# meyerls/FruitNeRF

Measured on AMD Instinct MI355X. Metric: train rays/sec, fruit_nerf on synthetic apple 800x800, higher is better.
Workload: dtype f32 fwd (MLP GEMMs: 3-piece bf16 split, 6 products, ~2^-24) / 2-piece bwd (dX, dW: 3 products, ~2^-17; its forward recompute 3-piece); everything else f32

## Files before the change

fruitnerf_amd/csrc/hash_scatter.hip:

```cpp
#include <stdlib.h>
#include <string.h>

#include "hash_sources.hpp"
#include "sequencer.hpp"

namespace fnr {

constexpr int SC_MAX_ROWS = 8192;
constexpr int SC_MAX_BINS = 256;
constexpr int SC_CHUNK = 512;
constexpr int SC_EMIT_THREADS = 512;
constexpr int SC_PER_THREAD = SC_CHUNK / SC_EMIT_THREADS;
constexpr int SC_BINS_PER_THREAD = 1;
static_assert(SC_MAX_BINS <= SC_EMIT_THREADS, "one bin per thread");
constexpr int SC_CNT_STRIDE = 32;

__device__ unsigned long long g_scatter_overflow_records;
__device__ unsigned long long g_scatter_records[2][64][16];



struct ScatterPlan {
  int log2_rows;
  int bins_per_level;
// ... 62 lines not shown
  const unsigned long long heads = __ballot(head);
  const uint32_t row = (uint32_t)(heads >> (lane & 48)) & 0xffffu;
  const uint32_t below = row & ((2u << j) - 1u);
  const int dist = j - (31 - __clz((int)below));
  RunMasks m;
  m.g1 = dist >= 1 ? 1.0f : 0.0f;
  m.g2 = dist >= 2 ? 1.0f : 0.0f;
  m.g4 = dist >= 4 ? 1.0f : 0.0f;
  m.g8 = dist >= 8 ? 1.0f : 0.0f;
  m.tail = (j == 15) || ((row >> (j + 1)) & 1u);
  m.any_run = ~heads != 0ull;
  return m;
}
__device__ __forceinline__ float run_sum(float v, const RunMasks& m) {
  v = fmaf(m.g1, dpp_shr0_f32<0x111>(v), v);
  v = fmaf(m.g2, dpp_shr0_f32<0x112>(v), v);
  v = fmaf(m.g4, dpp_shr0_f32<0x114>(v), v);
  v = fmaf(m.g8, dpp_shr0_f32<0x118>(v), v);
  return v;
}



template <class Source, bool PAIRS>
__global__ __launch_bounds__(SC_EMIT_THREADS) void k_scatter_emit(GridDev grid, Warp warp, Source src, long long N,
                                                      const float2* __restrict__ d_feats, float2* __restrict__ queue_v,
                                                      unsigned short* __restrict__ queue_r, unsigned* __restrict__ qcount, unsigned* __restrict__ qmax,
                                                      long long cap, int log2_rows, int level0, int level_count, int lpb
                                                      ) {
  __shared__ float2 s_val[SC_CHUNK * 8];
  __shared__ unsigned s_key[SC_CHUNK * 8];
  __shared__ unsigned s_cnt[SC_MAX_BINS];
  __shared__ unsigned s_off[SC_MAX_BINS];
  __shared__ unsigned s_base[SC_MAX_BINS];
  __shared__ unsigned s_max;
  __shared__ unsigned s_wsum[SC_EMIT_THREADS / 64];
  const int bins = 1 << (grid.log2_T - log2_rows);
  const int lane = threadIdx.x & 63, wave = threadIdx.x >> 6;
  const uint32_t mask = (1u << grid.log2_T) - 1u;
  const uint32_t row_mask = (1u << log2_rows) - 1u;
  const long long n0 = (long long)blockIdx.x * SC_CHUNK;
  static_assert(SC_PER_THREAD == 1, "one sample per thread");
  const long long n = n0 + threadIdx.x;
  const bool valid = n < N;
  float x[3] = {0.f, 0.f, 0.f};
  float2 gf_next = make_float2(0.f, 0.f);
  const int lrel0 = blockIdx.y * lpb;
  if (valid) {
    gf_next = ntc_load<NT_DFEATS_LD>(&d_feats[(size_t)(level0 + lrel0) * N + n]);
    float px, py, pz;
    src.position(n, px, py, pz);
    warp_position(warp, px, py, pz, x);
  }
  for (int li = 0; li < lpb && lrel0 + li < level_count; ++li) {
  const int lrel = lrel0 + li;
  const int level = level0 + lrel;
  for (int i = threadIdx.x; i < bins; i += SC_EMIT_THREADS) {
    s_cnt[i] = 0;
  }
  if (threadIdx.x == 0) s_max = 0;
  __syncthreads();
  const int scaling = grid.scalings[level];
  const float2 gf = gf_next;
  if (valid && li + 1 < lpb && lrel + 1 < level_count) gf_next = ntc_load<NT_DFEATS_LD>(&d_feats[(size_t)(level + 1) * N + n]);

  uint32_t hk[SC_PER_THREAD][8];
  float vxk[SC_PER_THREAD][8], vyk[SC_PER_THREAD][8];
  float tmax = 0.0f;
  unsigned emit_mask[SC_PER_THREAD];
#pragma unroll
// ... 110 lines not shown
  __syncthreads();
  float* table = reinterpret_cast<float*>(grid.table + ((size_t)level << grid.log2_T));
  unsigned overflowed_here = 0;
  for (unsigned i = threadIdx.x; i < total; i += SC_EMIT_THREADS) {
    const float2 v = s_val[i];
    const unsigned key = s_key[i];
    const unsigned bin = key >> 16, row_in_bin = key & 0xffffu;
    const unsigned slot = s_base[bin] + (i - s_off[bin]);
    if ((long long)slot < cap) {
      const size_t q = ((size_t)lrel * bins + bin) * cap + slot;
      queue_v[q] = v;
      queue_r[q] = (unsigned short)row_in_bin;
    } else {
      qmax[(size_t)lrel * SC_CNT_STRIDE + 1] = 1u;
      ++overflowed_here;
      const size_t row = ((size_t)bin << log2_rows) + row_in_bin;
      atomicAdd(table + 2 * row, v.x);
      atomicAdd(table + 2 * row + 1, v.y);
    }
  }
  if (overflowed_here) atomicAdd(&g_scatter_overflow_records, (unsigned long long)overflowed_here);
  __syncthreads();
  }
}

__device__ __forceinline__ void acc_record(unsigned long long* __restrict__ s_acc, unsigned row, const float2& v,
                                           double scale) {
  const long long ix = __double2ll_rn((double)v.x * scale), iy = __double2ll_rn((double)v.y * scale);
  atomicAdd(&s_acc[2 * row], (unsigned long long)ix);
  atomicAdd(&s_acc[2 * row + 1], (unsigned long long)iy);
}

struct AccArgs {
  GridDev grid;
  const float2* queue_v;
  const unsigned short* queue_r;
  unsigned *qcount, *qmax, *qdone;
  long long cap;
  int log2_rows, level0, nbins;
  int kind;
  TableAdam adam;
};

template <bool ADAM>
__device__ __forceinline__ void accumulate_bin(const AccArgs& A, int vblock, unsigned long long* __restrict__ s_acc) {
  const GridDev& grid = A.grid;
// ... 121 lines not shown
        const int pair = e2 >> 1;
        if (!((tw1[pair >> 5] >> (pair & 31)) & 1u)) atomicOr(&tw1[pair >> 5], 1u << (pair & 31));
      }
      float2 P = adam.p[row0 + e2], M = adam.m[row0 + e2], V = adam.v[row0 + e2];
      table_adam_update(adam, g.x, P.x, M.x, V.x);
      table_adam_update(adam, g.y, P.y, M.y, V.y);
      adam.p[row0 + e2] = P;
      adam.m[row0 + e2] = M;
      adam.v[row0 + e2] = V;
    }
  } else {
    for (int e2 = threadIdx.x; e2 < rows; e2 += blockDim.x) {
      const long long ax = (long long)s_acc[2 * e2], ay = (long long)s_acc[2 * e2 + 1];
      if (ax != 0 || ay != 0) {
        float2 t = dst[e2];
        t.x += (float)((double)ax * inv);
        t.y += (float)((double)ay * inv);
        dst[e2] = t;
      }
    }
  }
}

extern __shared__ __attribute__((aligned(16))) unsigned char acc_smem[];
template <bool ADAM>
__global__ __launch_bounds__(1024) void k_scatter_accumulate(AccArgs a) {
  accumulate_bin<ADAM>(a, (int)blockIdx.x, reinterpret_cast<unsigned long long*>(acc_smem));
}
template <bool ADAM>
__global__ __launch_bounds__(1024) void k_scatter_accumulate2(AccArgs a, AccArgs b) {
  unsigned long long* s_acc = reinterpret_cast<unsigned long long*>(acc_smem);
  if ((int)blockIdx.x < a.nbins) accumulate_bin<ADAM>(a, (int)blockIdx.x, s_acc);
  else accumulate_bin<ADAM>(b, (int)blockIdx.x - a.nbins, s_acc);
}


template <class Source>
static int scatter_emit(const fnr_grid* grid_grad, const Warp& warp, const Source& src, long long N,
                        const float2* d_feats, int level0, int level_count, void* workspace, size_t workspace_bytes,
                        int workspace_clean, hipStream_t st, const TableAdam* adam, AccArgs& acc) {
  FNR_CHECK_ARG(level0 >= 0 && level_count >= 1 && level0 + level_count <= grid_grad->n_levels,
                "hash scatter: level range [%d,+%d) outside the %d levels", level0, level_count, grid_grad->n_levels);
  const ScatterPlan p = scatter_plan(N, level_count, grid_grad->log2_hashmap_size);
  FNR_CHECK_ARG(p.bins_per_level <= SC_MAX_BINS, "hash scatter: log2_hashmap_size %d too large for the bin histogram",
                grid_grad->log2_hashmap_size);
  FNR_CHECK_ARG(workspace && workspace_bytes >= p.count_bytes + p.queue_bytes, "hash scatter: workspace too small");
  unsigned* qcount = reinterpret_cast<unsigned*>(workspace);
  float2* queue_v = reinterpret_cast<float2*>(reinterpret_cast<char*>(workspace) + p.count_bytes);
  unsigned short* queue_r = reinterpret_cast<unsigned short*>(reinterpret_cast<char*>(workspace) + p.count_bytes + p.value_bytes);
  if (!workspace_clean) FNR_HIP(hipMemsetAsync(qcount, 0, p.count_bytes, st));
  const size_t nbins_all = (size_t)level_count * p.bins_per_level;
  const long long chunks = (N + SC_CHUNK - 1) / SC_CHUNK;
  FNR_CHECK_ARG(chunks < (1ll << 31), "hash scatter: too many samples");
  const GridDev gd = make_grid(grid_grad);
  for (int l = 0; l < grid_grad->n_levels; ++l)
    FNR_CHECK_ARG(gd.scalings[l] > 0 && gd.scalings[l] < 65535, "hash scatter: level resolution %d out of range", gd.scalings[l]);
  bool pairs = true;
  for (int l = level0; l < level0 + level_count; ++l) pairs = pairs && gd.scalings[l] < (1 << p.log2_rows);
  int lpb = 1;
  {
    const char* e = getenv("FNR_EMIT_LPB");
    const int forced = e ? atoi(e) : 0;
    const long long slots = 3ll * device_cu_count();
    while (lpb < level_count && lpb < 8 && chunks * ((level_count + 2 * lpb - 1) / (2 * lpb)) >= 2 * slots) lpb *= 2;
    if (forced > 0) lpb = forced;
    if (lpb > level_count) lpb = level_count;
  }
  const unsigned gy = (unsigned)((level_count + lpb - 1) / lpb);
  if (chunks == 0) {
  } else if (pairs)
    hipLaunchKernelGGL((k_scatter_emit<Source, true>), dim3((unsigned)chunks, gy), dim3(SC_EMIT_THREADS),
                       0, st, gd, warp, src, N, d_feats, queue_v, queue_r, qcount, qcount + nbins_all * SC_CNT_STRIDE, p.cap,
                       p.log2_rows, level0, level_count, lpb);
  else
    hipLaunchKernelGGL((k_scatter_emit<Source, false>), dim3((unsigned)chunks, gy), dim3(SC_EMIT_THREADS),
                       0, st, gd, warp, src, N, d_feats, queue_v, queue_r, qcount, qcount + nbins_all * SC_CNT_STRIDE, p.cap,
                       p.log2_rows, level0, level_count, lpb);
  FNR_LAUNCH_CHECK();
  acc.grid = gd;
  acc.queue_v = queue_v, acc.queue_r = queue_r, acc.qcount = qcount;
  acc.qmax = qcount + nbins_all * SC_CNT_STRIDE;
  acc.qdone = qcount + (nbins_all + level_count) * SC_CNT_STRIDE;
  acc.cap = p.cap, acc.log2_rows = p.log2_rows, acc.level0 = level0;
  acc.nbins = level_count * p.bins_per_level;
  acc.kind = 0;
  acc.adam = adam ? *adam : TableAdam{};
  return FNR_OK;
}

static int acc_lds_bytes(const AccArgs& a) { return (2 << a.log2_rows) * (int)sizeof(unsigned long long); }

static int scatter_accumulate(const AccArgs& a, bool adam, hipStream_t st) {
  const int bytes = acc_lds_bytes(a);
  if (adam) {
    const int rc = ensure_dyn_lds<k_scatter_accumulate<true>>(2 * SC_MAX_ROWS * (int)sizeof(unsigned long long));
    if (rc) return rc;
    hipLaunchKernelGGL(k_scatter_accumulate<true>, dim3((unsigned)a.nbins), dim3(1024), bytes, st, a);
  } else {
    const int rc = ensure_dyn_lds<k_scatter_accumulate<false>>(2 * SC_MAX_ROWS * (int)sizeof(unsigned long long));
    if (rc) return rc;
    hipLaunchKernelGGL(k_scatter_accumulate<false>, dim3((unsigned)a.nbins), dim3(1024), bytes, st, a);
  }
  FNR_LAUNCH_CHECK();
  return FNR_OK;
}

static int scatter_accumulate2(const AccArgs& a, const AccArgs& b, bool adam, hipStream_t st) {
  const int bytes = acc_lds_bytes(a) > acc_lds_bytes(b) ? acc_lds_bytes(a) : acc_lds_bytes(b);
  if (adam) {
    const int rc = ensure_dyn_lds<k_scatter_accumulate2<true>>(2 * SC_MAX_ROWS * (int)sizeof(unsigned long long));
    if (rc) return rc;
    hipLaunchKernelGGL(k_scatter_accumulate2<true>, dim3((unsigned)(a.nbins + b.nbins)), dim3(1024), bytes, st, a, b);
  } else {
    const int rc = ensure_dyn_lds<k_scatter_accumulate2<false>>(2 * SC_MAX_ROWS * (int)sizeof(unsigned long long));
    if (rc) return rc;
    hipLaunchKernelGGL(k_scatter_accumulate2<false>, dim3((unsigned)(a.nbins + b.nbins)), dim3(1024), bytes, st, a, b);
  }
  FNR_LAUNCH_CHECK();
  return FNR_OK;
}

template <class Source>
static int binned_scatter(const fnr_grid* grid_grad, const Warp& warp, const Source& src, long long N,
                          const float2* d_feats, int level0, int level_count, void* workspace, size_t workspace_bytes,
                          int workspace_clean, hipStream_t st, const TableAdam* adam = nullptr) {
  AccArgs acc;
  const int rc = scatter_emit(grid_grad, warp, src, N, d_feats, level0, level_count, workspace, workspace_bytes,
                              workspace_clean, st, adam, acc);
  if (rc) return rc;
  return scatter_accumulate(acc, adam != nullptr, st);
}

constexpr int PROP_PART = 320;

template <int L, int H, bool POSGRAD>
__global__ __launch_bounds__(256) void k_prop_bwd(GridDev grid, float4* __restrict__ d_xw, Warp warp, RaySource src,
                                                  long long N, const float* __restrict__ w0,
                                                  const float* __restrict__ b0, const float* __restrict__ w1,
                                                  const float* __restrict__ b1, const float2* __restrict__ feat_save,
                                                  const float* __restrict__ d_density, float2* __restrict__ d_feats,
                                                  float* __restrict__ partials) {
  constexpr int K = 2 * L;
  __shared__ float s_dh[256][H + 1];
  __shared__ float s_ha[256][H + 1];
  __shared__ float s_f[256][K + 1];
  __shared__ float s_do[256];
  static_assert(H == 16 && K <= 16, "phase 2 is a single 16x16 MFMA tile");
  using f32x4 = __attribute__((ext_vector_type(4))) float;
  const int tid = threadIdx.x;
  const int lane = tid & 63, wave = tid >> 6;
  const int j = lane & 15, g = lane >> 4;
  f32x4 d1 = {0.f, 0.f, 0.f, 0.f}, d2 = {0.f, 0.f, 0.f, 0.f}, d3 = {0.f, 0.f, 0.f, 0.f};
  float db1 = 0.0f;
  const float ones_col0 = (j == 0) ? 1.0f : 0.0f;
  const long long n_iter = (N + 255) / 256;
  for (long long it = blockIdx.x; it < n_iter; it += gridDim.x) {
    const long long n = it * 256 + tid;
    float f[K], dout = 0.0f;
#pragma unroll
    for (int k = 0; k < K; ++k) f[k] = 0.0f;
    bool sel = false;
    float x[3] = {0.f, 0.f, 0.f};
    if (n < N) {
      float px, py, pz;
      src.position(n, px, py, pz);
      sel = warp_position(warp, px, py, pz, x);
#pragma unroll
      for (int l = 0; l < L; ++l) {
        const float2 v = ntc_load<NT_PROP_FEATS>(&feat_save[(size_t)l * N + n]);
        f[2 * l] = v.x;
        f[2 * l + 1] = v.y;
      }
    }
    float a[H];
    float out = b1[0];
#pragma unroll
    for (int o = 0; o < H; ++o) {
      float t = b0[o];
#pragma unroll
// ... 56 lines not shown
      const float bf = (j < K) ? s_f[row][j < K ? j : 0] : 0.0f;
      d1 = __builtin_amdgcn_mfma_f32_16x16x4f32(a1, bf, d1, 0, 0, 0);
      d2 = __builtin_amdgcn_mfma_f32_16x16x4f32(a2, ones_col0, d2, 0, 0, 0);
      d3 = __builtin_amdgcn_mfma_f32_16x16x4f32(a1, ones_col0, d3, 0, 0, 0);
    }
    __syncthreads();
  }
  float* red = &s_dh[0][0];
#pragma unroll
  for (int r = 0; r < 4; ++r) {
    red[((wave * 3 + 0) * 16 + 4 * g + r) * 16 + j] = d1[r];
    red[((wave * 3 + 1) * 16 + 4 * g + r) * 16 + j] = d2[r];
    red[((wave * 3 + 2) * 16 + 4 * g + r) * 16 + j] = d3[r];
  }
  db1 = wave_sum(db1);
  if (lane == 0) s_do[wave] = db1;
  __syncthreads();
  {
    const int o = tid >> 4, k = tid & 15;
    auto total = [&](int which) {
      return (red[((0 * 3 + which) * 16 + o) * 16 + k] + red[((1 * 3 + which) * 16 + o) * 16 + k]) +
             (red[((2 * 3 + which) * 16 + o) * 16 + k] + red[((3 * 3 + which) * 16 + o) * 16 + k]);
    };
    float* part = partials + (size_t)blockIdx.x * PROP_PART;
    part[tid] = total(0);
    if (k == 0) {
      part[256 + o] = total(1);
      part[272 + o] = total(2);
    }
    if (tid == 0) part[288] = (s_do[0] + s_do[1]) + (s_do[2] + s_do[3]);
  }
}

constexpr int PRD_E = 16, PRD_Y = 64;
struct PropReduceArgs {
  const float* partials;
  int nblocks, K;
  float *g_w0, *g_b0, *g_w1, *g_b1;
  WeightAdam wa;
};
template <bool ADAM>
__device__ __forceinline__ void prop_reduce_block(int block, const PropReduceArgs& a) {
  __shared__ float s_part[PRD_Y][PRD_E];
  const float* __restrict__ partials = a.partials;
  const int nblocks = a.nblocks, K = a.K;
  const int t = threadIdx.x % PRD_E, y = threadIdx.x / PRD_E;
  const int e = block * PRD_E + t;
  float s = 0.0f;
  if (e <= 288) {
    int b = y;
    for (; b + 7 * PRD_Y < nblocks; b += 8 * PRD_Y) {
      float v[8];
#pragma unroll
      for (int u = 0; u < 8; ++u) v[u] = partials[(size_t)(b + u * PRD_Y) * PROP_PART + e];
#pragma unroll
      for (int u = 0; u < 8; ++u) s += v[u];
    }
    for (; b < nblocks; b += PRD_Y) s += partials[(size_t)b * PROP_PART + e];
  }
  s_part[y][t] = s;
  __syncthreads();
  if (y != 0 || e > 288) return;
#pragma unroll 8
  for (int q = 1; q < PRD_Y; ++q) s += s_part[q][t];
  if (!ADAM && s == 0.0f) return;
  float* dst = nullptr;
  if (e < 256) {
    const int o = e >> 4, k = e & 15;
    if (k < K) dst = &a.g_w0[o * K + k];
  } else if (e < 272) {
    dst = &a.g_w1[e - 256];
  } else if (e < 288) {
    dst = &a.g_b0[e - 272];
  } else {
    dst = &a.g_b1[0];
  }
  if (!dst) return;
  if constexpr (ADAM) weight_adam_entry(a.wa, dst, s);
  else *dst += s;
}
template <bool ADAM>
__global__ __launch_bounds__(PRD_E * PRD_Y) void k_prop_reduce(PropReduceArgs a) {
  prop_reduce_block<ADAM>((int)blockIdx.x, a);
}
template <bool ADAM>
__global__ __launch_bounds__(PRD_E * PRD_Y) void k_prop_reduce2(PropReduceArgs a, PropReduceArgs b) {
  constexpr int NB = PROP_PART / PRD_E;
  if ((int)blockIdx.x < NB) prop_reduce_block<ADAM>((int)blockIdx.x, a);
  else prop_reduce_block<ADAM>((int)blockIdx.x - NB, b);
}

}

using namespace fnr;


extern "C" int fnr_debug_scatter_overflows(uint64_t* count_host, int reset) {
  FNR_CHECK_ARG(count_host, "debug_scatter_overflows: null argument");
  unsigned long long n = 0;
  FNR_HIP(hipMemcpyFromSymbol(&n, HIP_SYMBOL(g_scatter_overflow_records), sizeof(n)));
  *count_host = n;
  if (reset) {
    n = 0;
// ... 52 lines not shown
      const fnr_table_adam a = seq::patched(adam_, sc);
      return fnr_hash_encode_bwd_adam(&grid_, &warp_, &rays_, euclid_bins, S, d_feats, workspace, workspace_bytes,
                                      workspace_clean, &a, stream);
    });
  }
  FNR_CHECK_ARG(grid_grad && warp && rays && euclid_bins && d_feats && S > 0, "hash_encode_bwd_adam: null argument");
  FNR_CHECK_ARG(grid_grad->n_levels >= 1 && grid_grad->n_levels <= FNR_MAX_LEVELS, "hash_encode_bwd_adam: n_levels");
  TableAdam t;
  const int rc = make_table_adam(adam, t);
  if (rc) return rc;
  const long long N = rays->n_rays * (long long)S;
  RaySource src{make_rays(rays), euclid_bins, S};
  FNR_PROF(OP_ENCODE_BWD, N);
  return binned_scatter(grid_grad, make_warp(warp), src, N, reinterpret_cast<const float2*>(d_feats), 0,
                        grid_grad->n_levels, workspace, workspace_bytes, workspace_clean, as_stream(stream), &t);
}

extern "C" size_t fnr_prop_density_bwd_workspace_bytes(int64_t n_samples, int n_levels, int log2_hashmap_size) {
  const size_t dfeat = ((size_t)n_levels * (size_t)n_samples * sizeof(float2) + 255) / 256 * 256;
  const size_t partials = (size_t)3 * device_cu_count() * PROP_PART * sizeof(float);
  return dfeat + partials + fnr_hash_scatter_workspace_bytes(n_samples, n_levels, log2_hashmap_size);
}

static int prop_density_bwd_entry(const fnr_prop_net* net, const fnr_prop_net* grads, const fnr_warp* warp,
                                    const fnr_rays* rays, const float* euclid_bins, int S, const float* feat_save,
                                    const float* d_density, float* d_position, void* workspace,
                                    size_t workspace_bytes, int workspace_clean, void* stream,
                                    const fnr_table_adam* table_adam, const fnr_table_adam* weight_adam,
                                    const float* grad_arena, AccArgs* defer_acc = nullptr, int phase = 0,
                                    bool own_scope = true, PropReduceArgs* defer_reduce = nullptr) {
  FNR_CHECK_ARG(net && grads && warp && rays && euclid_bins && feat_save && d_density && workspace && S > 0,
                "prop_density_bwd: null argument");
  WeightAdam wa{};
  TableAdam ta;
  if (table_adam) {
    FNR_CHECK_ARG(weight_adam && grad_arena, "prop_density_bwd_adam: weight_adam / grad_arena missing");
    int rca = make_table_adam(weight_adam, wa.t);
    if (rca) return rca;
    wa.p_off = weight_adam->params - grad_arena;
    wa.m_off = weight_adam->exp_avg - grad_arena;
    wa.v_off = weight_adam->exp_avg_sq - grad_arena;
    rca = make_table_adam(table_adam, ta);
    if (rca) return rca;
  }
  FNR_UNSUPPORTED(net->hidden_dim == 16, "prop_density_bwd: hidden_dim %d not built (16 only)", net->hidden_dim);
  FNR_CHECK_ARG(grads->grid.table && grads->w0 && grads->b0 && grads->w1 && grads->b1,
                "prop_density_bwd: null gradient pointer");
  const long long N = rays->n_rays * (long long)S;
  if (N == 0) return FNR_OK;
  const int L = net->grid.n_levels;
  FNR_CHECK_ARG(workspace_bytes >= fnr_prop_density_bwd_workspace_bytes(N, L, net->grid.log2_hashmap_size),
                "prop_density_bwd: workspace too small");
  RaySource src{make_rays(rays), euclid_bins, S};
  long long blocks = (N + 255) / 256;
  const long long max_blocks = 3ll * device_cu_count();
  if (blocks > max_blocks) blocks = max_blocks;
  {
    static const int cap_per_cu = [] { const char* e = getenv("FNR_PROP_BWD_WGS_PER_CU"); const int v = e ? atoi(e) : 0; return (v >= 1 && v <= 3) ? v : 3; }();
    const long long capped = (long long)cap_per_cu * device_cu_count();
    if (blocks > capped) blocks = capped;
  }
  Warp w = make_warp(warp);
  const float2* fs = reinterpret_cast<const float2*>(feat_save);
  float2* d_feats = reinterpret_cast<float2*>(workspace);
  const size_t dfeat_bytes = ((size_t)L * (size_t)N * sizeof(float2) + 255) / 256 * 256;
  float* partials = reinterpret_cast<float*>(reinterpret_cast<char*>(workspace) + dfeat_bytes);
  const size_t partial_bytes = (size_t)max_blocks * PROP_PART * sizeof(float);
  ::fnr::ProfScope prof_scope__(own_scope ? (int)OP_PROP_BWD : -1, N, stream);
  if (phase != 2) {
  const GridDev pgrid = make_grid(&net->grid);
  float4* d_xw = reinterpret_cast<float4*>(d_position);
#define FNR_PROPB_CASE(LL)                                                                                          \
  case LL:                                                                                                          \
    if (d_xw)                                                                                                       \
      hipLaunchKernelGGL((k_prop_bwd<LL, 16, true>), dim3((unsigned)blocks), dim3(256), 0, as_stream(stream), pgrid, \
                         d_xw, w, src, N, net->w0, net->b0, net->w1, net->b1, fs, d_density, d_feats, partials);    \
    else                                                                                                            \
      hipLaunchKernelGGL((k_prop_bwd<LL, 16, false>), dim3((unsigned)blocks), dim3(256), 0, as_stream(stream), pgrid, \
                         d_xw, w, src, N, net->w0, net->b0, net->w1, net->b1, fs, d_density, d_feats, partials);    \
    break;
  switch (L) {
    FNR_PROPB_CASE(1)
    FNR_PROPB_CASE(2)
    FNR_PROPB_CASE(3)
    FNR_PROPB_CASE(4)
    FNR_PROPB_CASE(5)
    FNR_PROPB_CASE(6)
    FNR_PROPB_CASE(7)
    FNR_PROPB_CASE(8)
    default:
      FNR_UNSUPPORTED(false, "prop_density_bwd: n_levels %d not built (1..8)", L);
  }
#undef FNR_PROPB_CASE
  FNR_LAUNCH_CHECK();
  const PropReduceArgs ra{partials, (int)blocks, 2 * L, grads->w0, grads->b0, grads->w1, grads->b1, table_adam ? wa : WeightAdam{}};
  if (defer_reduce) {
    *defer_reduce = ra;
  } else {
    if (table_adam) hipLaunchKernelGGL(k_prop_reduce<true>, dim3(PROP_PART / PRD_E), dim3(PRD_E * PRD_Y), 0, as_stream(stream), ra);
    else hipLaunchKernelGGL(k_prop_reduce<false>, dim3(PROP_PART / PRD_E), dim3(PRD_E * PRD_Y), 0, as_stream(stream), ra);
    FNR_LAUNCH_CHECK();
  }
  }
  if (phase == 1) return FNR_OK;
  AccArgs acc;
  const int rce = scatter_emit(&grads->grid, w, src, N, d_feats, 0, L,
                               reinterpret_cast<char*>(workspace) + dfeat_bytes + partial_bytes,
                               workspace_bytes - dfeat_bytes - partial_bytes, workspace_clean, as_stream(stream),
                               table_adam ? &ta : nullptr, acc);
  if (rce) return rce;
  acc.kind = 1;
  if (defer_acc) {
    *defer_acc = acc;
    return FNR_OK;
  }
  return scatter_accumulate(acc, table_adam != nullptr, as_stream(stream));
}

extern "C" int fnr_prop_density_bwd(const fnr_prop_net* net, const fnr_prop_net* grads, const fnr_warp* warp,
                                    const fnr_rays* rays, const float* euclid_bins, int S, const float* feat_save,
                                    const float* d_density, float* d_position, void* workspace,
                                    size_t workspace_bytes, int workspace_clean, void* stream) {
  FNR_SEQ_UNRECORDABLE("fnr_prop_density_bwd");
  return prop_density_bwd_entry(net, grads, warp, rays, euclid_bins, S, feat_save, d_density, d_position, workspace,
                                workspace_bytes, workspace_clean, stream, nullptr, nullptr, nullptr);
}

extern "C" int fnr_prop_density_bwd_adam(const fnr_prop_net* net, const fnr_prop_net* grads, const fnr_warp* warp,
                                         const fnr_rays* rays, const float* euclid_bins, int S, const float* feat_save,
                                         const float* d_density, float* d_position, const fnr_table_adam* table_adam,
                                         const fnr_table_adam* weight_adam, const float* grad_arena, void* workspace,
                                         size_t workspace_bytes, int workspace_clean, void* stream) {
  FNR_SEQ_UNRECORDABLE("fnr_prop_density_bwd_adam");
  FNR_CHECK_ARG(table_adam && weight_adam && grad_arena, "prop_density_bwd_adam: optimiser descriptors missing");
  return prop_density_bwd_entry(net, grads, warp, rays, euclid_bins, S, feat_save, d_density, d_position, workspace,
                                workspace_bytes, workspace_clean, stream, table_adam, weight_adam, grad_arena);
}

extern "C" int fnr_prop_density_bwd_pair(const fnr_prop_net* const* nets, const fnr_prop_net* const* grads,
                                         const fnr_warp* const* warps, const fnr_rays* rays,
                                         const float* const* euclid_bins, const int* S, const float* const* feat_save,
                                         const float* const* d_density, float* const* d_position,
                                         const fnr_table_adam* const* table_adam, const fnr_table_adam* weight_adam,
                                         const float* grad_arena, void* const* workspace, const size_t* workspace_bytes,
                                         const int* workspace_clean, void* stream) {
  if (seq::recording() && nets && grads && warps && rays && euclid_bins && S && feat_save && d_density && d_position &&
      workspace && workspace_bytes && workspace_clean && nets[0] && nets[1] && grads[0] && grads[1] && warps[0] && warps[1]) {
    struct Pair {
      fnr_prop_net net[2], grad[2];
      fnr_warp warp[2];
      fnr_rays rays;
      const float* euclid[2];
      int S[2];
      const float* feat[2];
      const float* dd[2];
      float* dpos[2];
      fnr_table_adam tadam[2], wadam;
      bool has_adam;
      void* ws[2];
// ... 7 lines not shown
    }
    p.rays = *rays;
    p.has_adam = table_adam && table_adam[0] && table_adam[1] && weight_adam;
    if (p.has_adam) p.tadam[0] = *table_adam[0], p.tadam[1] = *table_adam[1], p.wadam = *weight_adam;
    seq::push("fnr_prop_density_bwd_pair", [=](const fnr_step_scalars* sc) {
      const fnr_prop_net* n_[2] = {&p.net[0], &p.net[1]};
      const fnr_prop_net* g_[2] = {&p.grad[0], &p.grad[1]};
      const fnr_warp* w_[2] = {&p.warp[0], &p.warp[1]};
      const fnr_table_adam t0 = seq::patched(p.tadam[0], sc), t1 = seq::patched(p.tadam[1], sc), wa = seq::patched(p.wadam, sc);
      const fnr_table_adam* t_[2] = {&t0, &t1};
      return fnr_prop_density_bwd_pair(n_, g_, w_, &p.rays, p.euclid, p.S, p.feat, p.dd, p.dpos, p.has_adam ? t_ : nullptr,
                      p.has_adam ? &wa : nullptr, grad_arena, p.ws, p.ws_bytes, p.ws_clean, stream);
    });
  }
  FNR_CHECK_ARG(nets && grads && warps && rays && euclid_bins && S && feat_save && d_density && d_position && workspace &&
                    workspace_bytes && workspace_clean,
                "prop_density_bwd_pair: null argument");
  FNR_CHECK_ARG(nets[0] != nets[1] && grads[0] != grads[1] && workspace[0] != workspace[1],
                "prop_density_bwd_pair: the two levels must have their own network, gradients and workspace");
  const bool adam = table_adam && table_adam[0] && table_adam[1];
  FNR_CHECK_ARG(adam || !(table_adam && (table_adam[0] || table_adam[1])), "prop_density_bwd_pair: one table_adam missing");
  if (rays->n_rays == 0) return FNR_OK;
  FNR_PROF(OP_PROP_BWD, rays->n_rays * ((long long)S[0] + (long long)S[1]));
  AccArgs acc[2];
  for (int q = 0; q < 2; ++q) {
    const int rc = prop_density_bwd_entry(nets[q], grads[q], warps[q], rays, euclid_bins[q], S[q], feat_save[q], d_density[q],
                                          d_position[q], workspace[q], workspace_bytes[q], workspace_clean[q], stream,
                                          adam ? table_adam[q] : nullptr, adam ? weight_adam : nullptr,
                                          adam ? grad_arena : nullptr, &acc[q], 0, false);
    if (rc) return rc;
  }
  const bool first_longer = (long long)S[0] >= (long long)S[1];
  return scatter_accumulate2(first_longer ? acc[0] : acc[1], first_longer ? acc[1] : acc[0], adam, as_stream(stream));
}

extern "C" int fnr_prop_density_bwd_pair_split(const fnr_prop_net* const* nets, const fnr_prop_net* const* grads,
                                               const fnr_warp* const* warps, const fnr_rays* rays,
                                               const float* const* euclid_bins, const int* S, const float* const* feat_save,
                                               const float* const* d_density, float* const* d_position,
                                               const fnr_table_adam* const* table_adam, const fnr_table_adam* weight_adam,
                                               const float* grad_arena, void* const* workspace, const size_t* workspace_bytes,
                                               const int* workspace_clean, void* stream, void* position_ready_event) {
  if (seq::recording() && nets && grads && warps && rays && euclid_bins && S && feat_save && d_density && d_position &&
      workspace && workspace_bytes && workspace_clean && nets[0] && nets[1] && grads[0] && grads[1] && warps[0] && warps[1]) {
    struct Pair {
      fnr_prop_net net[2], grad[2];
// ... 20 lines not shown
    if (p.has_adam) p.tadam[0] = *table_adam[0], p.tadam[1] = *table_adam[1], p.wadam = *weight_adam;
    seq::push("fnr_prop_density_bwd_pair_split", [=](const fnr_step_scalars* sc) {
      const fnr_prop_net* n_[2] = {&p.net[0], &p.net[1]};
      const fnr_prop_net* g_[2] = {&p.grad[0], &p.grad[1]};
      const fnr_warp* w_[2] = {&p.warp[0], &p.warp[1]};
      const fnr_table_adam t0 = seq::patched(p.tadam[0], sc), t1 = seq::patched(p.tadam[1], sc), wa = seq::patched(p.wadam, sc);
      const fnr_table_adam* t_[2] = {&t0, &t1};
      return fnr_prop_density_bwd_pair_split(n_, g_, w_, &p.rays, p.euclid, p.S, p.feat, p.dd, p.dpos, p.has_adam ? t_ : nullptr,
                      p.has_adam ? &wa : nullptr, grad_arena, p.ws, p.ws_bytes, p.ws_clean, stream, position_ready_event);
    });
  }
  FNR_CHECK_ARG(nets && grads && warps && rays && euclid_bins && S && feat_save && d_density && d_position && workspace &&
                    workspace_bytes && workspace_clean,
                "prop_density_bwd_pair_split: null argument");
  FNR_CHECK_ARG(nets[0] != nets[1] && grads[0] != grads[1] && workspace[0] != workspace[1],
                "prop_density_bwd_pair_split: the two levels must have their own network, gradients and workspace");
  const bool adam = table_adam && table_adam[0] && table_adam[1];
  FNR_CHECK_ARG(adam || !(table_adam && (table_adam[0] || table_adam[1])), "prop_density_bwd_pair_split: one table_adam missing");
  if (rays->n_rays == 0) {
    if (position_ready_event) FNR_HIP(hipEventRecord(reinterpret_cast<hipEvent_t>(position_ready_event), as_stream(stream)));
    return FNR_OK;
  }
  FNR_PROF(OP_PROP_BWD, rays->n_rays * ((long long)S[0] + (long long)S[1]));
  AccArgs acc[2];
  PropReduceArgs red[2];
  for (int phase = 1; phase <= 2; ++phase) {
    for (int q = 0; q < 2; ++q) {
      const int rc = prop_density_bwd_entry(nets[q], grads[q], warps[q], rays, euclid_bins[q], S[q], feat_save[q], d_density[q],
                                            d_position[q], workspace[q], workspace_bytes[q], workspace_clean[q], stream,
                                            adam ? table_adam[q] : nullptr, adam ? weight_adam : nullptr,
                                            adam ? grad_arena : nullptr, &acc[q], phase, false, phase == 1 ? &red[q] : nullptr);
      if (rc) return rc;
    }
    if (phase == 1) {
      if (position_ready_event) FNR_HIP(hipEventRecord(reinterpret_cast<hipEvent_t>(position_ready_event), as_stream(stream)));
      constexpr unsigned NB = PROP_PART / PRD_E;
      if (adam) hipLaunchKernelGGL(k_prop_reduce2<true>, dim3(2 * NB), dim3(PRD_E * PRD_Y), 0, as_stream(stream), red[0], red[1]);
      else hipLaunchKernelGGL(k_prop_reduce2<false>, dim3(2 * NB), dim3(PRD_E * PRD_Y), 0, as_stream(stream), red[0], red[1]);
      FNR_LAUNCH_CHECK();
    }
  }
  const bool first_longer = (long long)S[0] >= (long long)S[1];
  return scatter_accumulate2(first_longer ? acc[0] : acc[1], first_longer ? acc[1] : acc[0], adam, as_stream(stream));
}
```

Baseline: 6.008 million.

## Merge paired proposal-net backward launches into combined bwd, emit and accumulate kernels

For the two proposal networks, the backward MLP kernels of both levels now run as one launch with block-range roles, and so do the two scatter-emit kernels. The weight-gradient reduce is folded into the scatter-accumulate kernel as extra workgroups. This cuts the chain from about seven launches to three and lets the smaller level's blocks fill idle CUs next to the larger one. The cost is more register and LDS pressure in the combined kernels (the accumulate kernel now also carries the reduce's shared arrays), and an env var can turn it off.

```diff
diff --git a/fruitnerf_amd/csrc/hash_scatter.hip b/fruitnerf_amd/csrc/hash_scatter.hip
--- a/fruitnerf_amd/csrc/hash_scatter.hip
+++ b/fruitnerf_amd/csrc/hash_scatter.hip
@@ -108,12 +108,27 @@
 
 
 
+template <class Source>
+struct EmitArgs {
+  GridDev grid;
+  Warp warp;
+  Source src;
+  long long N;
+  const float2* d_feats;
+  float2* queue_v;
+  unsigned short* queue_r;
+  unsigned *qcount, *qmax;
+  long long cap;
+  int log2_rows, level0, level_count, lpb;
+  unsigned chunks, gy;
+};
 template <class Source, bool PAIRS>
-__global__ __launch_bounds__(SC_EMIT_THREADS) void k_scatter_emit(GridDev grid, Warp warp, Source src, long long N,
-                                                      const float2* __restrict__ d_feats, float2* __restrict__ queue_v,
-                                                      unsigned short* __restrict__ queue_r, unsigned* __restrict__ qcount, unsigned* __restrict__ qmax,
-                                                      long long cap, int log2_rows, int level0, int level_count, int lpb
-                                                      ) {
+__device__ __forceinline__ void scatter_emit_block(const GridDev& grid, const Warp& warp, const Source& src, const long long N,
+                                                   const float2* __restrict__ d_feats, float2* __restrict__ queue_v,
+                                                   unsigned short* __restrict__ queue_r, unsigned* __restrict__ qcount,
+                                                   unsigned* __restrict__ qmax, const long long cap, const int log2_rows,
+                                                   const int level0, const int level_count, const int lpb, const unsigned bx,
+                                                   const unsigned by) {
   __shared__ float2 s_val[SC_CHUNK * 8];
   __shared__ unsigned s_key[SC_CHUNK * 8];
   __shared__ unsigned s_cnt[SC_MAX_BINS];
@@ -125,13 +140,13 @@
   const int lane = threadIdx.x & 63, wave = threadIdx.x >> 6;
   const uint32_t mask = (1u << grid.log2_T) - 1u;
   const uint32_t row_mask = (1u << log2_rows) - 1u;
-  const long long n0 = (long long)blockIdx.x * SC_CHUNK;
+  const long long n0 = (long long)bx * SC_CHUNK;
   static_assert(SC_PER_THREAD == 1, "one sample per thread");
   const long long n = n0 + threadIdx.x;
   const bool valid = n < N;
   float x[3] = {0.f, 0.f, 0.f};
   float2 gf_next = make_float2(0.f, 0.f);
-  const int lrel0 = blockIdx.y * lpb;
+  const int lrel0 = (int)by * lpb;
   if (valid) {
     gf_next = ntc_load<NT_DFEATS_LD>(&d_feats[(size_t)(level0 + lrel0) * N + n]);
     float px, py, pz;
@@ -288,6 +303,25 @@
   if (overflowed_here) atomicAdd(&g_scatter_overflow_records, (unsigned long long)overflowed_here);
   __syncthreads();
   }
+}
+template <class Source, bool PAIRS>
+__global__ __launch_bounds__(SC_EMIT_THREADS) void k_scatter_emit(EmitArgs<Source> a) {
+  scatter_emit_block<Source, PAIRS>(a.grid, a.warp, a.src, a.N, a.d_feats, a.queue_v, a.queue_r, a.qcount, a.qmax, a.cap,
+                                    a.log2_rows, a.level0, a.level_count, a.lpb, blockIdx.x, blockIdx.y);
+}
+template <class Source>
+struct EmitArgs2 {
+  EmitArgs<Source> c[2];
+};
+template <class Source, bool PAIRS>
+__global__ __launch_bounds__(SC_EMIT_THREADS) void k_scatter_emit2(EmitArgs2<Source> p) {
+  const unsigned first = p.c[0].chunks * p.c[0].gy;
+  const int role = blockIdx.x >= first ? 1 : 0;
+  const EmitArgs<Source>& a = p.c[role];
+  const unsigned r = blockIdx.x - (role ? first : 0u);
+  const unsigned by = r / a.chunks, bx = r - by * a.chunks;
+  scatter_emit_block<Source, PAIRS>(a.grid, a.warp, a.src, a.N, a.d_feats, a.queue_v, a.queue_r, a.qcount, a.qmax, a.cap,
+                                    a.log2_rows, a.level0, a.level_count, a.lpb, bx, by);
 }
 
 __device__ __forceinline__ void acc_record(unsigned long long* __restrict__ s_acc, unsigned row, const float2& v,
@@ -455,23 +489,112 @@
   }
 }
 
+constexpr int PROP_PART = 320;
+constexpr int PRD_E = 16, PRD_Y = 64;
+struct PropReduceArgs {
+  const float* partials;
+  int nblocks, K;
+  float *g_w0, *g_b0, *g_w1, *g_b1;
+  WeightAdam wa;
+};
+template <bool ADAM>
+__device__ __forceinline__ void prop_reduce_block(int block, const PropReduceArgs& a) {
+  __shared__ float s_part[PRD_Y][PRD_E];
+  const float* __restrict__ partials = a.partials;
+  const int nblocks = a.nblocks, K = a.K;
+  const int t = threadIdx.x % PRD_E, y = threadIdx.x / PRD_E;
+  const int e = block * PRD_E + t;
+  float s = 0.0f;
+  if (e <= 288) {
+    int b = y;
+    for (; b + 7 * PRD_Y < nblocks; b += 8 * PRD_Y) {
+      float v[8];
+#pragma unroll
+      for (int u = 0; u < 8; ++u) v[u] = partials[(size_t)(b + u * PRD_Y) * PROP_PART + e];
+#pragma unroll
+      for (int u = 0; u < 8; ++u) s += v[u];
+    }
+    for (; b < nblocks; b += PRD_Y) s += partials[(size_t)b * PROP_PART + e];
+  }
+  s_part[y][t] = s;
+  __syncthreads();
+  if (y != 0 || e > 288) return;
+#pragma unroll 8
+  for (int q = 1; q < PRD_Y; ++q) s += s_part[q][t];
+  if (!ADAM && s == 0.0f) return;
+  float* dst = nullptr;
+  if (e < 256) {
+    const int o = e >> 4, k = e & 15;
+    if (k < K) dst = &a.g_w0[o * K + k];
+  } else if (e < 272) {
+    dst = &a.g_w1[e - 256];
+  } else if (e < 288) {
+    dst = &a.g_b0[e - 272];
+  } else {
+    dst = &a.g_b1[0];
+  }
+  if (!dst) return;
+  if constexpr (ADAM) weight_adam_entry(a.wa, dst, s);
+  else *dst += s;
+}
+
 extern __shared__ __attribute__((aligned(16))) unsigned char acc_smem[];
 template <bool ADAM>
 __global__ __launch_bounds__(1024) void k_scatter_accumulate(AccArgs a) {
   accumulate_bin<ADAM>(a, (int)blockIdx.x, reinterpret_cast<unsigned long long*>(acc_smem));
 }
+static_assert(PRD_E * PRD_Y == 1024, "the reduce role runs in the accumulate kernel's workgroups");
 template <bool ADAM>
-__global__ __launch_bounds__(1024) void k_scatter_accumulate2(AccArgs a, AccArgs b) {
+__global__ __launch_bounds__(1024) void k_scatter_accumulate2(AccArgs a, AccArgs b, PropReduceArgs ra, PropReduceArgs rb) {
   unsigned long long* s_acc = reinterpret_cast<unsigned long long*>(acc_smem);
+  constexpr int NB = PROP_PART / PRD_E;
+  const int r = (int)blockIdx.x - a.nbins - b.nbins;
   if ((int)blockIdx.x < a.nbins) accumulate_bin<ADAM>(a, (int)blockIdx.x, s_acc);
-  else accumulate_bin<ADAM>(b, (int)blockIdx.x - a.nbins, s_acc);
-}
-
+  else if (r < 0) accumulate_bin<ADAM>(b, (int)blockIdx.x - a.nbins, s_acc);
+  else if (r < NB) prop_reduce_block<ADAM>(r, ra);
+  else prop_reduce_block<ADAM>(r - NB, rb);
+}
+
+
+template <class Source>
+struct EmitLaunch {
+  EmitArgs<Source> args;
+  bool pairs;
+};
+template <class Source>
+static int scatter_emit_launch(const EmitLaunch<Source>& e, hipStream_t st) {
+  const EmitArgs<Source>& a = e.args;
+  if (a.chunks == 0) {
+  } else if (e.pairs)
+    hipLaunchKernelGGL((k_scatter_emit<Source, true>), dim3(a.chunks, a.gy), dim3(SC_EMIT_THREADS), 0, st, a);
+  else
+    hipLaunchKernelGGL((k_scatter_emit<Source, false>), dim3(a.chunks, a.gy), dim3(SC_EMIT_THREADS), 0, st, a);
+  FNR_LAUNCH_CHECK();
+  return FNR_OK;
+}
+template <class Source>
+static int scatter_emit2(const EmitLaunch<Source>& x, const EmitLaunch<Source>& y, hipStream_t st) {
+  const unsigned long long nx = (unsigned long long)x.args.chunks * x.args.gy, ny = (unsigned long long)y.args.chunks * y.args.gy;
+  if (x.pairs != y.pairs || nx == 0 || ny == 0 || nx + ny >= (1ull << 31)) {
+    const int rc = scatter_emit_launch(x, st);
+    if (rc) return rc;
+    return scatter_emit_launch(y, st);
+  }
+  EmitArgs2<Source> p;
+  const bool x_first = x.args.N >= y.args.N;
+  p.c[0] = x_first ? x.args : y.args;
+  p.c[1] = x_first ? y.args : x.args;
+  if (x.pairs) hipLaunchKernelGGL((k_scatter_emit2<Source, true>), dim3((unsigned)(nx + ny)), dim3(SC_EMIT_THREADS), 0, st, p);
+  else hipLaunchKernelGGL((k_scatter_emit2<Source, false>), dim3((unsigned)(nx + ny)), dim3(SC_EMIT_THREADS), 0, st, p);
+  FNR_LAUNCH_CHECK();
+  return FNR_OK;
+}
 
 template <class Source>
 static int scatter_emit(const fnr_grid* grid_grad, const Warp& warp, const Source& src, long long N,
                         const float2* d_feats, int level0, int level_count, void* workspace, size_t workspace_bytes,
-                        int workspace_clean, hipStream_t st, const TableAdam* adam, AccArgs& acc) {
+                        int workspace_clean, hipStream_t st, const TableAdam* adam, AccArgs& acc,
+                        EmitLaunch<Source>* defer = nullptr) {
   FNR_CHECK_ARG(level0 >= 0 && level_count >= 1 && level0 + level_count <= grid_grad->n_levels,
                 "hash scatter: level range [%d,+%d) outside the %d levels", level0, level_count, grid_grad->n_levels);
   const ScatterPlan p = scatter_plan(N, level_count, grid_grad->log2_hashmap_size);
@@ -500,16 +623,16 @@
     if (lpb > level_count) lpb = level_count;
   }
   const unsigned gy = (unsigned)((level_count + lpb - 1) / lpb);
-  if (chunks == 0) {
-  } else if (pairs)
-    hipLaunchKernelGGL((k_scatter_emit<Source, true>), dim3((unsigned)chunks, gy), dim3(SC_EMIT_THREADS),
-                       0, st, gd, warp, src, N, d_feats, queue_v, queue_r, qcount, qcount + nbins_all * SC_CNT_STRIDE, p.cap,
-                       p.log2_rows, level0, level_count, lpb);
-  else
-    hipLaunchKernelGGL((k_scatter_emit<Source, false>), dim3((unsigned)chunks, gy), dim3(SC_EMIT_THREADS),
-                       0, st, gd, warp, src, N, d_feats, queue_v, queue_r, qcount, qcount + nbins_all * SC_CNT_STRIDE, p.cap,
-                       p.log2_rows, level0, level_count, lpb);
-  FNR_LAUNCH_CHECK();
+  const EmitArgs<Source> ea{gd, warp, src, N, d_feats, queue_v, queue_r, qcount, qcount + nbins_all * SC_CNT_STRIDE, p.cap,
+                            p.log2_rows, level0, level_count, lpb, (unsigned)chunks, gy};
+  FNR_CHECK_ARG(chunks * gy < (1ll << 31), "hash scatter: too many samples");
+  if (defer) {
+    defer->args = ea;
+    defer->pairs = pairs;
+  } else {
+    const int rc = scatter_emit_launch(EmitLaunch<Source>{ea, pairs}, st);
+    if (rc) return rc;
+  }
   acc.grid = gd;
   acc.queue_v = queue_v, acc.queue_r = queue_r, acc.qcount = qcount;
   acc.qmax = qcount + nbins_all * SC_CNT_STRIDE;
@@ -538,16 +661,19 @@
   return FNR_OK;
 }
 
-static int scatter_accumulate2(const AccArgs& a, const AccArgs& b, bool adam, hipStream_t st) {
+static int scatter_accumulate2(const AccArgs& a, const AccArgs& b, bool adam, hipStream_t st,
+                               const PropReduceArgs* red = nullptr) {
   const int bytes = acc_lds_bytes(a) > acc_lds_bytes(b) ? acc_lds_bytes(a) : acc_lds_bytes(b);
+  const unsigned grid = (unsigned)(a.nbins + b.nbins) + (red ? 2u * (PROP_PART / PRD_E) : 0u);
+  const PropReduceArgs ra = red ? red[0] : PropReduceArgs{}, rb = red ? red[1] : PropReduceArgs{};
   if (adam) {
     const int rc = ensure_dyn_lds<k_scatter_accumulate2<true>>(2 * SC_MAX_ROWS * (int)sizeof(unsigned long long));
     if (rc) return rc;
-    hipLaunchKernelGGL(k_scatter_accumulate2<true>, dim3((unsigned)(a.nbins + b.nbins)), dim3(1024), bytes, st, a, b);
+    hipLaunchKernelGGL(k_scatter_accumulate2<true>, dim3(grid), dim3(1024), bytes, st, a, b, ra, rb);
   } else {
     const int rc = ensure_dyn_lds<k_scatter_accumulate2<false>>(2 * SC_MAX_ROWS * (int)sizeof(unsigned long long));
     if (rc) return rc;
-    hipLaunchKernelGGL(k_scatter_accumulate2<false>, dim3((unsigned)(a.nbins + b.nbins)), dim3(1024), bytes, st, a, b);
+    hipLaunchKernelGGL(k_scatter_accumulate2<false>, dim3(grid), dim3(1024), bytes, st, a, b, ra, rb);
   }
   FNR_LAUNCH_CHECK();
   return FNR_OK;
@@ -564,15 +690,26 @@
   return scatter_accumulate(acc, adam != nullptr, st);
 }
 
-constexpr int PROP_PART = 320;
-
+struct PropBwdArgs {
+  GridDev grid;
+  float4* d_xw;
+  Warp warp;
+  RaySource src;
+  long long N;
+  const float *w0, *b0, *w1, *b1;
+  const float2* feat_save;
+  const float* d_density;
+  float2* d_feats;
+  float* partials;
+  int blocks;
+};
 template <int L, int H, bool POSGRAD>
-__global__ __launch_bounds__(256) void k_prop_bwd(GridDev grid, float4* __restrict__ d_xw, Warp warp, RaySource src,
-                                                  long long N, const float* __restrict__ w0,
-                                                  const float* __restrict__ b0, const float* __restrict__ w1,
-                                                  const float* __restrict__ b1, const float2* __restrict__ feat_save,
-                                                  const float* __restrict__ d_density, float2* __restrict__ d_feats,
-                                                  float* __restrict__ partials) {
+__device__ __forceinline__ void prop_bwd_block(const GridDev& grid, float4* __restrict__ d_xw, const Warp& warp,
+                                               const RaySource& src, const long long N, const float* __restrict__ w0,
+                                               const float* __restrict__ b0, const float* __restrict__ w1,
+                                               const float* __restrict__ b1, const float2* __restrict__ feat_save,
+                                               const float* __restrict__ d_density, float2* __restrict__ d_feats,
+                                               float* __restrict__ partials, const int block, const int nblocks) {
   constexpr int K = 2 * L;
   __shared__ float s_dh[256][H + 1];
   __shared__ float s_ha[256][H + 1];
@@ -587,7 +724,7 @@
   float db1 = 0.0f;
   const float ones_col0 = (j == 0) ? 1.0f : 0.0f;
   const long long n_iter = (N + 255) / 256;
-  for (long long it = blockIdx.x; it < n_iter; it += gridDim.x) {
+  for (long long it = block; it < n_iter; it += nblocks) {
     const long long n = it * 256 + tid;
     float f[K], dout = 0.0f;
 #pragma unroll
@@ -690,7 +827,7 @@
       return (red[((0 * 3 + which) * 16 + o) * 16 + k] + red[((1 * 3 + which) * 16 + o) * 16 + k]) +
              (red[((2 * 3 + which) * 16 + o) * 16 + k] + red[((3 * 3 + which) * 16 + o) * 16 + k]);
     };
-    float* part = partials + (size_t)blockIdx.x * PROP_PART;
+    float* part = partials + (size_t)block * PROP_PART;
     part[tid] = total(0);
     if (k == 0) {
       part[256 + o] = total(1);
@@ -699,54 +836,22 @@
     if (tid == 0) part[288] = (s_do[0] + s_do[1]) + (s_do[2] + s_do[3]);
   }
 }
-
-constexpr int PRD_E = 16, PRD_Y = 64;
-struct PropReduceArgs {
-  const float* partials;
-  int nblocks, K;
-  float *g_w0, *g_b0, *g_w1, *g_b1;
-  WeightAdam wa;
+template <int L, int H, bool POSGRAD>
+__global__ __launch_bounds__(256) void k_prop_bwd(PropBwdArgs a) {
+  prop_bwd_block<L, H, POSGRAD>(a.grid, a.d_xw, a.warp, a.src, a.N, a.w0, a.b0, a.w1, a.b1, a.feat_save, a.d_density, a.d_feats,
+                                a.partials, (int)blockIdx.x, (int)gridDim.x);
+}
+struct PropBwdArgs2 {
+  PropBwdArgs c[2];
 };
-template <bool ADAM>
-__device__ __forceinline__ void prop_reduce_block(int block, const PropReduceArgs& a) {
-  __shared__ float s_part[PRD_Y][PRD_E];
-  const float* __restrict__ partials = a.partials;
-  const int nblocks = a.nblocks, K = a.K;
-  const int t = threadIdx.x % PRD_E, y = threadIdx.x / PRD_E;
-  const int e = block * PRD_E + t;
-  float s = 0.0f;
-  if (e <= 288) {
-    int b = y;
-    for (; b + 7 * PRD_Y < nblocks; b += 8 * PRD_Y) {
-      float v[8];
-#pragma unroll
-      for (int u = 0; u < 8; ++u) v[u] = partials[(size_t)(b + u * PRD_Y) * PROP_PART + e];
-#pragma unroll
-      for (int u = 0; u < 8; ++u) s += v[u];
-    }
-    for (; b < nblocks; b += PRD_Y) s += partials[(size_t)b * PROP_PART + e];
-  }
-  s_part[y][t] = s;
-  __syncthreads();
-  if (y != 0 || e > 288) return;
-#pragma unroll 8
-  for (int q = 1; q < PRD_Y; ++q) s += s_part[q][t];
-  if (!ADAM && s == 0.0f) return;
-  float* dst = nullptr;
-  if (e < 256) {
-    const int o = e >> 4, k = e & 15;
-    if (k < K) dst = &a.g_w0[o * K + k];
-  } else if (e < 272) {
-    dst = &a.g_w1[e - 256];
-  } else if (e < 288) {
-    dst = &a.g_b0[e - 272];
-  } else {
-    dst = &a.g_b1[0];
-  }
-  if (!dst) return;
-  if constexpr (ADAM) weight_adam_entry(a.wa, dst, s);
-  else *dst += s;
-}
+template <int L, int H, bool POSGRAD>
+__global__ __launch_bounds__(256) void k_prop_bwd2(PropBwdArgs2 p) {
+  const int role = (int)blockIdx.x >= p.c[0].blocks ? 1 : 0;
+  const PropBwdArgs& a = p.c[role];
+  prop_bwd_block<L, H, POSGRAD>(a.grid, a.d_xw, a.warp, a.src, a.N, a.w0, a.b0, a.w1, a.b1, a.feat_save, a.d_density, a.d_feats,
+                                a.partials, (int)blockIdx.x - (role ? p.c[0].blocks : 0), a.blocks);
+}
+
 template <bool ADAM>
 __global__ __launch_bounds__(PRD_E * PRD_Y) void k_prop_reduce(PropReduceArgs a) {
   prop_reduce_block<ADAM>((int)blockIdx.x, a);
@@ -845,13 +950,69 @@
   return dfeat + partials + fnr_hash_scatter_workspace_bytes(n_samples, n_levels, log2_hashmap_size);
 }
 
+static int prop_bwd_launch(const PropBwdArgs& a, int L, hipStream_t st) {
+#define FNR_PROPB_CASE(LL)                                                                                        \
+  case LL:                                                                                                        \
+    if (a.d_xw) hipLaunchKernelGGL((k_prop_bwd<LL, 16, true>), dim3((unsigned)a.blocks), dim3(256), 0, st, a);     \
+    else hipLaunchKernelGGL((k_prop_bwd<LL, 16, false>), dim3((unsigned)a.blocks), dim3(256), 0, st, a);          \
+    break;
+  switch (L) {
+    FNR_PROPB_CASE(1)
+    FNR_PROPB_CASE(2)
+    FNR_PROPB_CASE(3)
+    FNR_PROPB_CASE(4)
+    FNR_PROPB_CASE(5)
+    FNR_PROPB_CASE(6)
+    FNR_PROPB_CASE(7)
+    FNR_PROPB_CASE(8)
+    default:
+      FNR_UNSUPPORTED(false, "prop_density_bwd: n_levels %d not built (1..8)", L);
+  }
+#undef FNR_PROPB_CASE
+  FNR_LAUNCH_CHECK();
+  return FNR_OK;
+}
+static int prop_bwd_launch2(const PropBwdArgs& x, int Lx, const PropBwdArgs& y, int Ly, hipStream_t st) {
+  if (Lx != Ly || (x.d_xw != nullptr) != (y.d_xw != nullptr)) {
+    const int rc = prop_bwd_launch(x, Lx, st);
+    if (rc) return rc;
+    return prop_bwd_launch(y, Ly, st);
+  }
+  PropBwdArgs2 p;
+  const bool x_first = x.N >= y.N;
+  p.c[0] = x_first ? x : y;
+  p.c[1] = x_first ? y : x;
+  const unsigned grid = (unsigned)(x.blocks + y.blocks);
+#define FNR_PROPB2_CASE(LL)                                                                                 \
+  case LL:                                                                                                  \
+    if (x.d_xw) hipLaunchKernelGGL((k_prop_bwd2<LL, 16, true>), dim3(grid), dim3(256), 0, st, p);            \
+    else hipLaunchKernelGGL((k_prop_bwd2<LL, 16, false>), dim3(grid), dim3(256), 0, st, p);                 \
+    break;
+  switch (Lx) {
+    FNR_PROPB2_CASE(1)
+    FNR_PROPB2_CASE(2)
+    FNR_PROPB2_CASE(3)
+    FNR_PROPB2_CASE(4)
+    FNR_PROPB2_CASE(5)
+    FNR_PROPB2_CASE(6)
+    FNR_PROPB2_CASE(7)
+    FNR_PROPB2_CASE(8)
+    default:
+      FNR_UNSUPPORTED(false, "prop_density_bwd: n_levels %d not built (1..8)", Lx);
+  }
+#undef FNR_PROPB2_CASE
+  FNR_LAUNCH_CHECK();
+  return FNR_OK;
+}
+
 static int prop_density_bwd_entry(const fnr_prop_net* net, const fnr_prop_net* grads, const fnr_warp* warp,
                                     const fnr_rays* rays, const float* euclid_bins, int S, const float* feat_save,
                                     const float* d_density, float* d_position, void* workspace,
                                     size_t workspace_bytes, int workspace_clean, void* stream,
                                     const fnr_table_adam* table_adam, const fnr_table_adam* weight_adam,
                                     const float* grad_arena, AccArgs* defer_acc = nullptr, int phase = 0,
-                                    bool own_scope = true, PropReduceArgs* defer_reduce = nullptr) {
+                                    bool own_scope = true, PropReduceArgs* defer_reduce = nullptr,
+                                    PropBwdArgs* defer_bwd = nullptr, EmitLaunch<RaySource>* defer_emit = nullptr) {
   FNR_CHECK_ARG(net && grads && warp && rays && euclid_bins && feat_save && d_density && workspace && S > 0,
                 "prop_density_bwd: null argument");
   WeightAdam wa{};
@@ -893,29 +1054,14 @@
   if (phase != 2) {
   const GridDev pgrid = make_grid(&net->grid);
   float4* d_xw = reinterpret_cast<float4*>(d_position);
-#define FNR_PROPB_CASE(LL)                                                                                          \
-  case LL:                                                                                                          \
-    if (d_xw)                                                                                                       \
-      hipLaunchKernelGGL((k_prop_bwd<LL, 16, true>), dim3((unsigned)blocks), dim3(256), 0, as_stream(stream), pgrid, \
-                         d_xw, w, src, N, net->w0, net->b0, net->w1, net->b1, fs, d_density, d_feats, partials);    \
-    else                                                                                                            \
-      hipLaunchKernelGGL((k_prop_bwd<LL, 16, false>), dim3((unsigned)blocks), dim3(256), 0, as_stream(stream), pgrid, \
-                         d_xw, w, src, N, net->w0, net->b0, net->w1, net->b1, fs, d_density, d_feats, partials);    \
-    break;
-  switch (L) {
-    FNR_PROPB_CASE(1)
-    FNR_PROPB_CASE(2)
-    FNR_PROPB_CASE(3)
-    FNR_PROPB_CASE(4)
-    FNR_PROPB_CASE(5)
-    FNR_PROPB_CASE(6)
-    FNR_PROPB_CASE(7)
-    FNR_PROPB_CASE(8)
-    default:
-      FNR_UNSUPPORTED(false, "prop_density_bwd: n_levels %d not built (1..8)", L);
-  }
-#undef FNR_PROPB_CASE
-  FNR_LAUNCH_CHECK();
+  const PropBwdArgs ba{pgrid, d_xw, w, src, N, net->w0, net->b0, net->w1, net->b1, fs, d_density, d_feats, partials, (int)blocks};
+  FNR_UNSUPPORTED(L >= 1 && L <= 8, "prop_density_bwd: n_levels %d not built (1..8)", L);
+  if (defer_bwd) {
+    *defer_bwd = ba;
+  } else {
+    const int rcl = prop_bwd_launch(ba, L, as_stream(stream));
+    if (rcl) return rcl;
+  }
   const PropReduceArgs ra{partials, (int)blocks, 2 * L, grads->w0, grads->b0, grads->w1, grads->b1, table_adam ? wa : WeightAdam{}};
   if (defer_reduce) {
     *defer_reduce = ra;
@@ -930,7 +1076,7 @@
   const int rce = scatter_emit(&grads->grid, w, src, N, d_feats, 0, L,
                                reinterpret_cast<char*>(workspace) + dfeat_bytes + partial_bytes,
                                workspace_bytes - dfeat_bytes - partial_bytes, workspace_clean, as_stream(stream),
-                               table_adam ? &ta : nullptr, acc);
+                               table_adam ? &ta : nullptr, acc, defer_emit);
   if (rce) return rce;
   acc.kind = 1;
   if (defer_acc) {
@@ -958,6 +1104,43 @@
   FNR_CHECK_ARG(table_adam && weight_adam && grad_arena, "prop_density_bwd_adam: optimiser descriptors missing");
   return prop_density_bwd_entry(net, grads, warp, rays, euclid_bins, S, feat_save, d_density, d_position, workspace,
                                 workspace_bytes, workspace_clean, stream, table_adam, weight_adam, grad_arena);
+}
+
+static bool prop_chain_merged() {
+  const char* e = getenv("FNR_PROP_CHAIN_MERGED");
+  return !(e && e[0] == '0' && e[1] == 0);
+}
+
+static int prop_pair_merged(const fnr_prop_net* const* nets, const fnr_prop_net* const* grads, const fnr_warp* const* warps,
+                            const fnr_rays* rays, const float* const* euclid_bins, const int* S,
+                            const float* const* feat_save, const float* const* d_density, float* const* d_position,
+                            const fnr_table_adam* const* table_adam, const fnr_table_adam* weight_adam,
+                            const float* grad_arena, void* const* workspace, const size_t* workspace_bytes,
+                            const int* workspace_clean, void* stream, void* position_ready_event, bool adam) {
+  AccArgs acc[2];
+  PropReduceArgs red[2];
+  PropBwdArgs bwd[2];
+  EmitLaunch<RaySource> emit[2];
+  for (int phase = 1; phase <= 2; ++phase) {
+    for (int q = 0; q < 2; ++q) {
+      const int rc = prop_density_bwd_entry(nets[q], grads[q], warps[q], rays, euclid_bins[q], S[q], feat_save[q], d_density[q],
+                                            d_position[q], workspace[q], workspace_bytes[q], workspace_clean[q], stream,
+                                            adam ? table_adam[q] : nullptr, adam ? weight_adam : nullptr,
+                                            adam ? grad_arena : nullptr, &acc[q], phase, false, phase == 1 ? &red[q] : nullptr,
+                                            phase == 1 ? &bwd[q] : nullptr, phase == 2 ? &emit[q] : nullptr);
+      if (rc) return rc;
+    }
+    if (phase == 1) {
+      const int rc = prop_bwd_launch2(bwd[0], nets[0]->grid.n_levels, bwd[1], nets[1]->grid.n_levels, as_stream(stream));
+      if (rc) return rc;
+      if (position_ready_event) FNR_HIP(hipEventRecord(reinterpret_cast<hipEvent_t>(position_ready_event), as_stream(stream)));
+    } else {
+      const int rc = scatter_emit2(emit[0], emit[1], as_stream(stream));
+      if (rc) return rc;
+    }
+  }
+  const bool first_longer = (long long)S[0] >= (long long)S[1];
+  return scatter_accumulate2(first_longer ? acc[0] : acc[1], first_longer ? acc[1] : acc[0], adam, as_stream(stream), red);
 }
 
 extern "C" int fnr_prop_density_bwd_pair(const fnr_prop_net* const* nets, const fnr_prop_net* const* grads,
@@ -1011,6 +1194,9 @@
   FNR_CHECK_ARG(adam || !(table_adam && (table_adam[0] || table_adam[1])), "prop_density_bwd_pair: one table_adam missing");
   if (rays->n_rays == 0) return FNR_OK;
   FNR_PROF(OP_PROP_BWD, rays->n_rays * ((long long)S[0] + (long long)S[1]));
+  if (prop_chain_merged())
+    return prop_pair_merged(nets, grads, warps, rays, euclid_bins, S, feat_save, d_density, d_position, table_adam, weight_adam,
+                            grad_arena, workspace, workspace_bytes, workspace_clean, stream, nullptr, adam);
   AccArgs acc[2];
   for (int q = 0; q < 2; ++q) {
     const int rc = prop_density_bwd_entry(nets[q], grads[q], warps[q], rays, euclid_bins[q], S[q], feat_save[q], d_density[q],
@@ -1077,6 +1263,9 @@
     return FNR_OK;
   }
   FNR_PROF(OP_PROP_BWD, rays->n_rays * ((long long)S[0] + (long long)S[1]));
+  if (prop_chain_merged())
+    return prop_pair_merged(nets, grads, warps, rays, euclid_bins, S, feat_save, d_density, d_position, table_adam, weight_adam,
+                            grad_arena, workspace, workspace_bytes, workspace_clean, stream, position_ready_event, adam);
   AccArgs acc[2];
   PropReduceArgs red[2];
   for (int phase = 1; phase <= 2; ++phase) {
```

Measured after the change: 6.072 million, median of 6. 1.01x the previous value.
